# dash-robotics/perception

Measured on AMD Instinct MI355X. Metric: frames/sec (640x480 D435 cloud, plane+cluster+ICP), higher is better.
Workload: dtype f32

## Files before the change

### include/cuboid_hip.h

```cpp
#ifndef CUBOID_HIP_H
#define CUBOID_HIP_H

#include <stddef.h>
#include <stdint.h>

#ifdef __cplusplus
extern "C" {
#endif

#define CD_ABI_VERSION 4
#define CD_MAX_TEMPLATES 8
#define CD_MAX_CLUSTERS_PER_FRAME 8
#define CD_FRAME_MORE_CLUSTERS 1
#define CD_FRAME_SURFACE_GUESS 2
#define CD_FRAME_CLUSTER_GUESS 4

typedef struct cd_context cd_context;

typedef enum cd_status {
    CD_OK = 0,
    CD_ERR_INVALID_ARG = -1,
    CD_ERR_CAPACITY = -2,
    CD_ERR_DEVICE = -3,
    CD_ERR_NO_MODEL = -4,
// ... 66 lines not shown
    int32_t n_clusters;
    int32_t ransac_iterations;
    int32_t flags;
    float plane[4];
    float pad[4];
    cd_cluster_result clusters[CD_MAX_CLUSTERS_PER_FRAME];
} cd_frame_result;

void cd_default_params(cd_params* p);
int cd_abi_version(void);
int cd_struct_size(int which);

int cd_create(int device_id, int max_points, int max_frames, cd_context** out);
void cd_destroy(cd_context* ctx);
const char* cd_last_error(const cd_context* ctx);

int cd_set_template(cd_context* ctx, int slot, const void* xyz, size_t stride_bytes, int m);

int cd_template_lattice_faces(const cd_context* ctx, int slot);

int cd_template_nearest(cd_context* ctx, int slot, const void* queries, size_t stride_bytes, int n, int32_t* out_index,
                        float* out_d2);

int cd_lattice_detect(const void* xyz, size_t stride_bytes, int m, int32_t* out);

int cd_lattice_axes(const void* xyz, size_t stride_bytes, int m, int32_t* out_axis_face, float* out_axis_c);

int cd_crop_voxel(cd_context* ctx, const void* points, size_t stride_bytes, int n,
                  const cd_params* prm, float* out_xyz, uint32_t* out_rgb, int capacity,
                  int* out_n_cropped, int* out_n_voxels);

int cd_passthrough(cd_context* ctx, const void* points, size_t stride_bytes, int n, int field, double limit_min,
                   double limit_max, int negative, void* out_points, int capacity, int* out_n);

int cd_segment_plane(cd_context* ctx, const void* xyz, size_t stride_bytes, int n,
                     const cd_params* prm, float coeff[4], int32_t* inliers, int capacity,
                     int* out_n_inliers, int* out_iterations);

int cd_surface_frame(cd_context* ctx, const void* xyz, size_t stride_bytes, int n, const float table_normal[3],
                     int invert, const cd_params* prm, cd_surface_frame_result* out);

int cd_surface_batch(cd_context* ctx, const void* xyz, size_t stride_bytes, int points_per_frame, const int32_t* n_points,
                     int n_frames, const float* table_normals, int invert, const cd_params* prm, cd_surface_frame_result* out,
                     int32_t* frame_status);

int cd_surface_guess(const float Rt[16], float guess[16]);
// ... 235 lines not shown
```

### perception_amd/capi.py

```python
import ctypes as C
import os

import numpy as np

CD_ABI_VERSION = 4
CD_MAX_TEMPLATES = 8
CD_MAX_CLUSTERS_PER_FRAME = 8
CD_FRAME_MORE_CLUSTERS = 1
CD_FRAME_SURFACE_GUESS = 2
CD_FRAME_CLUSTER_GUESS = 4

CD_OK = 0
CD_ERR_INVALID_ARG = -1
CD_ERR_CAPACITY = -2
CD_ERR_DEVICE = -3
CD_ERR_NO_MODEL = -4
CD_ERR_FEW_CORRESPONDENCES = -5
CD_ERR_LEAF_TOO_SMALL = -6
CD_ERR_NO_TEMPLATE = -7

LIB_PATH = os.environ.get("CUBOID_HIP_LIB") or os.path.join(os.path.dirname(os.path.abspath(__file__)), "lib", "libcuboid_hip.so")

EXPORTED_SYMBOLS = [
    "cd_default_params", "cd_abi_version", "cd_struct_size", "cd_create", "cd_destroy", "cd_last_error",
    "cd_set_template", "cd_crop_voxel", "cd_segment_plane", "cd_extract", "cd_surface_frame", "cd_bbox_filter", "cd_cluster", "cd_icp",
    "cd_process_batch", "cd_process_frame", "cd_process_batch_device", "cd_get_cluster_results", "cd_pose_to_position_quaternion",
    "cd_bbox_corners", "cd_get_timing", "cd_get_frame_cloud", "cd_get_cluster_points", "cd_ground_plane", "cd_set_frame_guesses",
    "cd_template_lattice_faces", "cd_template_nearest", "cd_lattice_detect", "cd_lattice_axes", "cd_passthrough",
    "cd_default_depth_camera", "cd_depth_to_cloud", "cd_process_depth_batch", "cd_process_depth_batch_device",
    "cd_set_icp_max_correspondence_distance", "cd_get_icp_max_correspondence_distance", "cd_icp_correspondence_threshold",
    "cd_surface_batch", "cd_surface_guess", "cd_set_surface_distance_threshold", "cd_get_surface_distance_threshold",
    "cd_get_surface_results",
    "cd_default_color_gate_params", "cd_color_bbox_batch", "cd_color_bbox_batch_device", "cd_set_frame_bboxes", "cd_set_bbox_source",
    "cd_get_bbox_source", "cd_get_frame_bboxes",
    "cd_default_overlay_params", "cd_overlay_project", "cd_draw_boxes_batch", "cd_draw_boxes_batch_device", "cd_draw_last_results",
    "cd_draw_last_results_device",
    "cd_default_verify_params", "cd_verify_struct_size", "cd_verify_pixel", "cd_verify_box_host", "cd_verify_boxes_batch",
    "cd_verify_boxes_batch_device", "cd_verify_last_results", "cd_verify_last_results_device",
    "cd_default_color_camera", "cd_color_camera_struct_size", "cd_texture_project", "cd_depth_to_cloud_mapped",
    "cd_process_depth_batch_mapped", "cd_process_depth_batch_mapped_device",
    "cd_shape_frame_struct_size", "cd_shape_frame_host", "cd_shape_frames", "cd_template_shape_frame", "cd_shape_guess",
    "cd_get_cluster_shape_frames",
]

CD_CLOUD_VOXELS, CD_CLOUD_OBJECTS = 0, 1
CD_GUESS_NONE, CD_GUESS_PARAMS, CD_GUESS_PER_FRAME, CD_GUESS_SURFACE, CD_GUESS_CLUSTER = 0, 1, 2, 3, 4


CD_PLANE, CD_PLANE_PERPENDICULAR, CD_PLANE_PARALLEL = 0, 1, 2
CD_COLOR_NONE, CD_COLOR_RGB8 = 0, 1
CD_BBOX_PARAMS, CD_BBOX_PER_FRAME, CD_BBOX_COLOR = 0, 1, 2
CD_DRAW_ACCEPTED, CD_DRAW_ALL = 0, 1
CD_VERIFY_ACCEPTED, CD_VERIFY_ALL = 0, 1
CD_VERIFY_MISS, CD_VERIFY_AGREE, CD_VERIFY_THROUGH, CD_VERIFY_OCCLUDED, CD_VERIFY_INVALID = 0, 1, 2, 3, 4
CD_NOTEX_DROP, CD_NOTEX_KEEP = 0, 1


class CdSurfaceFrameResult(C.Structure):
    _fields_ = [("Rt", C.c_float * 16), ("coeff", (C.c_float * 4) * 3), ("midpoint", (C.c_float * 4) * 3),
                ("n_points", C.c_int32 * 3), ("iterations", C.c_int32 * 3), ("reserved", C.c_int32 * 2)]


class CdShapeFrame(C.Structure):
    _fields_ = [("n", C.c_int32), ("status", C.c_int32), ("mean", C.c_double * 3), ("axes", C.c_double * 9),
                ("var", C.c_double * 3), ("lo", C.c_double * 3), ("hi", C.c_double * 3)]
# ... 261 lines not shown
    lib.cd_icp.argtypes = [vp, C.c_int, vp, C.c_size_t, C.c_int, C.POINTER(CdParams),
                           C.POINTER(CdClusterResult), vp]
    for f in (lib.cd_process_batch, lib.cd_process_batch_device):
        f.argtypes = [vp, vp, C.c_size_t, C.c_int, C.c_int, C.POINTER(CdParams), vp, vp, vp]
    lib.cd_process_frame.argtypes = [vp, vp, C.c_size_t, C.c_int, C.POINTER(CdParams), vp, vp, vp]
    lib.cd_get_cluster_results.argtypes = [vp, C.c_int, C.c_int, C.c_int, C.POINTER(CdClusterResult), ip]
    lib.cd_pose_to_position_quaternion.argtypes = [C.POINTER(C.c_double)] * 3
    lib.cd_pose_to_position_quaternion.restype = None
    lib.cd_bbox_corners.argtypes = [C.POINTER(C.c_double), C.c_double, C.c_double, C.c_double, f32p]
    lib.cd_bbox_corners.restype = None
    lib.cd_get_timing.argtypes = [vp, C.POINTER(CdTiming)]
    lib.cd_get_frame_cloud.argtypes = [vp, C.c_int, C.c_int, vp, C.c_size_t, C.c_int, C.c_int, ip]
    lib.cd_get_cluster_points.argtypes = [vp, C.c_int, C.c_int, C.c_int, vp, C.c_size_t, C.c_int, ip]
    lib.cd_ground_plane.argtypes = [vp, vp, C.c_size_t, C.c_int, C.POINTER(CdParams), f32p, vp, C.c_int, ip, ip]
    lib.cd_set_frame_guesses.argtypes = [vp, f32p, C.c_int]
    lib.cd_surface_batch.argtypes = [vp, vp, C.c_size_t, C.c_int, i32p, C.c_int, f32p, C.c_int, C.POINTER(CdParams),
                                     C.POINTER(CdSurfaceFrameResult), i32p]
    lib.cd_surface_guess.argtypes = [f32p, f32p]
    lib.cd_set_surface_distance_threshold.argtypes = [vp, C.c_double]
    lib.cd_get_surface_distance_threshold.argtypes = [vp, C.POINTER(C.c_double)]
    lib.cd_get_surface_results.argtypes = [vp, C.c_int, C.c_int, C.POINTER(CdSurfaceFrameResult), i32p]
    lib.cd_template_lattice_faces.argtypes = [vp, C.c_int]
    lib.cd_template_nearest.argtypes = [vp, C.c_int, vp, C.c_size_t, C.c_int, vp, vp]
    lib.cd_lattice_detect.argtypes = [vp, C.c_size_t, C.c_int, vp]
    lib.cd_lattice_axes.argtypes = [vp, C.c_size_t, C.c_int, vp, vp]
    lib.cd_set_icp_max_correspondence_distance.argtypes = [vp, C.c_double]
    lib.cd_get_icp_max_correspondence_distance.argtypes = [vp, C.POINTER(C.c_double)]
    lib.cd_icp_correspondence_threshold.argtypes = [C.c_double, C.POINTER(C.c_float), ip]
    lib.cd_passthrough.argtypes = [vp, vp, C.c_size_t, C.c_int, C.c_int, C.c_double, C.c_double, C.c_int, vp, C.c_int, ip]
    lib.cd_default_depth_camera.argtypes = [C.POINTER(CdDepthCamera)]
    lib.cd_default_depth_camera.restype = None
    lib.cd_depth_to_cloud.argtypes = [vp, C.POINTER(CdDepthCamera), vp, vp, vp, C.c_size_t, C.c_int, C.c_int, ip]
    for f in (lib.cd_process_depth_batch, lib.cd_process_depth_batch_device):
        f.argtypes = [vp, C.POINTER(CdDepthCamera), vp, vp, C.c_int, C.POINTER(CdParams), vp, vp, vp]
    lib.cd_default_color_gate_params.argtypes = [C.POINTER(CdColorGateParams)]
    lib.cd_default_color_gate_params.restype = None
    for f in (lib.cd_color_bbox_batch, lib.cd_color_bbox_batch_device):
        f.argtypes = [vp, vp, C.c_int, C.c_int, C.c_int, C.POINTER(CdColorGateParams), C.POINTER(CdColorBBox)]
    lib.cd_set_frame_bboxes.argtypes = [vp, i32p, C.c_int]
    lib.cd_set_bbox_source.argtypes = [vp, C.c_int, C.POINTER(CdColorGateParams)]
    lib.cd_get_bbox_source.argtypes = [vp, ip]
    lib.cd_get_frame_bboxes.argtypes = [vp, C.c_int, C.c_int, C.POINTER(CdColorBBox)]
    dp = C.POINTER(C.c_double)
    lib.cd_default_overlay_params.argtypes = [C.POINTER(CdOverlayParams)]
    lib.cd_default_overlay_params.restype = None
    lib.cd_overlay_project.argtypes = [dp, C.POINTER(CdOverlayParams), C.POINTER(CdOverlayBox)]
# ... 467 lines not shown


def lattice_detect(xyz):
    lib = load_library()
    a, stride, m = _points(xyz)
    out = np.zeros((8, 5), np.int32)
    nf = lib.cd_lattice_detect(_ptr(a), stride, m, _ptr(out))
    if nf < 0:
        raise CuboidError(nf, "cd_lattice_detect")
    return [tuple(int(v) for v in out[f]) for f in range(nf)]


def lattice_axes(xyz):
    lib = load_library()
    a, stride, m = _points(xyz)
    face = np.zeros(3, np.int32)
    c = np.zeros(3, np.float32)
    r = lib.cd_lattice_axes(_ptr(a), stride, m, _ptr(face), _ptr(c))
    if r < 0:
        raise CuboidError(r, "cd_lattice_axes")
    return int(r), [int(v) for v in face], c


def icp_correspondence_threshold(d):
    lib = load_library()
    f, b = C.c_float(), C.c_int()
    st = lib.cd_icp_correspondence_threshold(float("inf") if d is None else float(d), C.byref(f), C.byref(b))
    if st != CD_OK:
        raise CuboidError(st, "cd_icp_correspondence_threshold")
    return f.value, int(b.value)


def surface_guess(Rt):
    lib = load_library()
    a = np.ascontiguousarray(Rt, np.float32).reshape(16)
    g = np.zeros(16, np.float32)
    f32 = C.POINTER(C.c_float)
    st = lib.cd_surface_guess(a.ctypes.data_as(f32), g.ctypes.data_as(f32))
    if st != CD_OK:
        raise CuboidError(st, "cd_surface_guess: non-finite input")
    return g.reshape(4, 4)


def shape_frame_host(xyz):
    lib = load_library()
    a = np.asarray(xyz, np.float32)
# ... 82 lines not shown
```

### perception_amd/csrc/entries.hip

```cpp
#include "context.hpp"
#include "host_math.hpp"

namespace {
int cd_crop_voxel_impl(cd_context* c, const void* points, size_t stride, int n, const cd_params* p, float* out_xyz,
                  uint32_t* out_rgb, int capacity, int* out_n_cropped, int* out_n_voxels) {
    invalidate_last(c);
    int st = check_params(c, p);
    if (st) return st;
    if (!points || !out_xyz || n < 0 || stride < 12 || (stride & 3)) return fail(c, CD_ERR_INVALID_ARG, "bad arguments");
    if (n > c->N) return fail(c, CD_ERR_CAPACITY, "more points than the context capacity");
    if (out_n_cropped) *out_n_cropped = 0;
    if (out_n_voxels) *out_n_voxels = 0;
    if (n == 0) return CD_OK;
    st = ensure_input(c, (size_t)n * stride);
    if (st) return st;
    HIPCHK(c, hipMemcpyAsync(c->d_in, points, (size_t)n * stride, hipMemcpyHostToDevice, c->stream));
    st = stage_crop_voxel(c, c->d_in, stride, n, 1, p, nullptr);
    if (st) return st;
    st = sync_fs(c, 1);
    if (st) return st;
    const FrameState& s = c->h_fs[0];
    if (out_n_cropped) *out_n_cropped = s.n_cropped;
    if (s.status != CD_OK) return fail(c, s.status, "voxel grid: leaf size too small for the input extent");
    if (s.n_v > capacity) return fail(c, CD_ERR_CAPACITY, "output capacity too small");
// ... 411 lines not shown
}
int cd_bbox_filter(cd_context* c, const void* xyz, size_t stride, int n, const double P[12], const int32_t rect[4], int32_t* out_indices, int capacity, int* out_n) {
    return with_scan_retry(c, [&] { return cd_bbox_filter_impl(c, xyz, stride, n, P, rect, out_indices, capacity, out_n); });
}
int cd_extract(cd_context* c, const void* points, size_t stride, int n, const int32_t* indices, int n_indices, int negative, void* out_points, int capacity, int* out_n) {
    return with_scan_retry(c, [&] { return cd_extract_impl(c, points, stride, n, indices, n_indices, negative, out_points, capacity, out_n); });
}
int cd_passthrough(cd_context* c, const void* points, size_t stride, int n, int field, double limit_min, double limit_max, int negative, void* out_points, int capacity, int* out_n) {
    return with_scan_retry(c, [&] { return cd_passthrough_impl(c, points, stride, n, field, limit_min, limit_max, negative, out_points, capacity, out_n); });
}
int cd_cluster(cd_context* c, const void* xyz, size_t stride, int n, const cd_params* p, int32_t* labels, int32_t* sizes, int sizes_capacity, int* out_k) {
    return with_scan_retry(c, [&] { return cd_cluster_impl(c, xyz, stride, n, p, labels, sizes, sizes_capacity, out_k); });
}
int cd_icp(cd_context* c, int slot, const void* src_xyz, size_t stride, int n, const cd_params* p, cd_cluster_result* out, float* aligned) {
    return with_scan_retry(c, [&] { return cd_icp_impl(c, slot, src_xyz, stride, n, p, out, aligned); });
}
int cd_shape_frames(cd_context* c, const void* xyz, size_t stride, const int32_t* offsets, int n_sets, cd_shape_frame* out) {
    return with_scan_retry(c, [&] { return cd_shape_frames_impl(c, xyz, stride, offsets, n_sets, out); });
}
int cd_ground_plane(cd_context* c, const void* points, size_t stride, int n, const cd_params* p, float coeff[4], void* out_records, int capacity, int* out_n, int* out_n_inliers) {
    return with_scan_retry(c, [&] { return cd_ground_plane_impl(c, points, stride, n, p, coeff, out_records, capacity, out_n, out_n_inliers); });
}
}
```

### perception_amd/csrc/k_icp_lat.hip

```cpp
#include "kernels.hpp"
#include "icp_solve.hpp"

namespace cd {

struct LatFaces {
    int nface;
    unsigned m0[LAT_MAX_FACES], m1[LAT_MAX_FACES], m2[LAT_MAX_FACES];
    float c[LAT_MAX_FACES];
    int nx, ny, nz, tox, toy, toz;
    float ox, oy, oz, ivx, ivy, ivz;
    int axes;
    int afx, afy, afz;
    float cax, cay, caz;
};

__device__ __forceinline__ void lat_faces_load(const IcpLattice* __restrict__ L, LatFaces& F) {
    F.nface = L->nface;
#pragma unroll
    for (int f = 0; f < LAT_MAX_FACES; ++f) { F.m0[f] = L->m0[f]; F.m1[f] = L->m1[f]; F.m2[f] = L->m2[f]; F.c[f] = L->c[f]; }
    F.nx = L->n[0]; F.ny = L->n[1]; F.nz = L->n[2]; F.tox = L->toff[0]; F.toy = L->toff[1]; F.toz = L->toff[2];
    F.ox = L->noi[0]; F.oy = L->noi[1]; F.oz = L->noi[2]; F.ivx = L->inv[0]; F.ivy = L->inv[1]; F.ivz = L->inv[2];
    F.axes = L->axes_distinct;
    F.afx = L->axis_face[0]; F.afy = L->axis_face[1]; F.afz = L->axis_face[2];
    asm("v_mov_b32 %0, %1" : "=v"(F.cax) : "s"(L->axis_c[0]));
// ... 201 lines not shown
#else
#define LAT_T(k)
#endif

template <int SHIFT>
struct LatFix {
    static constexpr unsigned long long C = ((unsigned long long)(1023 + 52 - SHIFT) << 52) | (1ull << 51);
    static __device__ __forceinline__ unsigned long long bits(float v) {
        return (unsigned long long)__double_as_longlong(__dadd_rn((double)v, __longlong_as_double((long long)C)));
    }
};
static_assert(LatFix<32>::C == 0x4138000000000000ull && LatFix<36>::C == 0x40f8000000000000ull, "constants of lat_fix");
static_assert(FIX_SHIFT == 32 && FIX_SHIFT_D2 == 36, "k_icp_lat's moment sums are written for these scales");

struct LatSlot {
    int k, src_off, n, tslot;
    int phase;
    int gen;
    int ready;
    int pad;
};
enum { LAT_ITER = 0, LAT_FIT = 1, LAT_EMPTY = 2 };

#ifndef CD_LAT_WAVES_PER_EU
#define CD_LAT_WAVES_PER_EU 4
#endif
template <int CPW, int WPC, bool BOUNDED>
__global__ void __launch_bounds__(CPW * WPC * WAVE, CD_LAT_WAVES_PER_EU)
k_icp_lat(int nitems, const int* __restrict__ order, const IcpCluster* __restrict__ cl, IcpState* __restrict__ st,
          unsigned long long* __restrict__ accf, const IcpLattice* __restrict__ lats, float4* __restrict__ src,
          const float4* __restrict__ src0, int* __restrict__ queue, unsigned long long* __restrict__ busy,
          unsigned long long* __restrict__ busy_out, IcpParams prm, IcpBound bnd) {
    __shared__ float4 s_tab[CPW][LAT_MAX_TAB];
    __shared__ int4 s_face[CPW][2 * LAT_MAX_FACES];
    __shared__ unsigned long long s_acc[CPW][16];
    __shared__ IcpState s_so[CPW];
    __shared__ LatSlot s_slot[CPW];
    __shared__ int s_flags[2];
    __shared__ unsigned s_nv[BOUNDED ? CPW : 1];
    const int lane = threadIdx.x & 63, wave = threadIdx.x >> 6;
    const int slot = wave / WPC, sub = wave % WPC;
    const long long wg_t0 = wall_clock64();
    auto refill = [&](int s) {
        LatSlot& sl = s_slot[s];
        for (int i = 0; i < 16; ++i) s_acc[s][i] = 0ull;
        if constexpr (BOUNDED) s_nv[s] = 0u;
// ... 110 lines not shown
                unsigned long long S[16];
#pragma unroll
                for (int i = 0; i < 16; ++i) S[i] = 0ull;
                float4 pnext = pts[min((sub << 6) + lane, n - 1)], p0next = pts0[min((sub << 6) + lane, n - 1)];
                for (int pss = sub; pss < npass; pss += WPC) {
                    const int myq = (pss << 6) + lane;
                    const bool act = myq < n;
                    const float4 p = pnext, p0 = p0next;
                    pnext = pts[min(((pss + WPC) << 6) + lane, n - 1)];
                    p0next = pts0[min(((pss + WPC) << 6) + lane, n - 1)];
                    float ox, oy, oz;
                    xform(T, p.x, p.y, p.z, ox, oy, oz);
                    if (act) pts[myq] = make_float4(ox, oy, oz, p.w);
                    float qx, qy, qz;
                    xform(Tf, p0.x, p0.y, p0.z, qx, qy, qz);
                    const LatHit h = F.axes ? lat_nearest_axes<false>(tab, face, F, qx, qy, qz)
                                            : (nf3 ? lat_nearest<false, 3>(tab, face, F, qx, qy, qz) : lat_nearest<false, LAT_MAX_FACES>(tab, face, F, qx, qy, qz));
                    if (act) S[0] += h.d < 16384.f ? LatFix<FIX_SHIFT_D2>::bits(h.d) : (unsigned long long)fixq(h.d, FIX_SHIFT_D2) + LatFix<FIX_SHIFT_D2>::C;
                }
                if (sub < npass) wave_fold_to_lds(S, 1, s_acc[slot]);
            }
        }
        LAT_T(0)
        __syncthreads();
        LAT_T(1)
        if (threadIdx.x == 0) s_flags[1] = 0;
        if (threadIdx.x < CPW) {
            const int s = threadIdx.x;
            LatSlot& sl = s_slot[s];
            const int nv = BOUNDED && sl.phase == LAT_ITER ? (int)s_nv[s] : sl.n;
            const unsigned long long off = (unsigned long long)nv * LatFix<FIX_SHIFT>::C, off_d = (unsigned long long)nv * LatFix<FIX_SHIFT_D2>::C;
            if (sl.phase == LAT_ITER && sl.ready) {
                for (int i = 0; i < 15; ++i) s_acc[s][i] -= off;
                s_acc[s][15] -= off_d;
                if (icp_step<BOUNDED>(s_so[s], s_acc[s], nv, prm)) sl.phase = LAT_FIT;
                for (int i = 0; i < 16; ++i) s_acc[s][i] = 0ull;
                if constexpr (BOUNDED) s_nv[s] = 0u;
                sl.ready = 0;
            } else if (sl.phase == LAT_FIT) {
                s_so[s].done = 1;
                st[2 * (size_t)sl.k] = s_so[s];
                st[2 * (size_t)sl.k + 1] = s_so[s];
                accf[sl.k] = s_acc[s][0] - off_d;
                refill(s);
                if (sl.phase != LAT_EMPTY) s_flags[1] = 1;
            }
        }
        if (threadIdx.x == 0) {
            int all_empty = 1;
            for (int s = 0; s < CPW; ++s) all_empty &= s_slot[s].phase == LAT_EMPTY ? 1 : 0;
            s_flags[0] = all_empty;
        }
        LAT_T(2)
        __syncthreads();
        LAT_T(3)
#ifdef CD_LAT_TIMERS
        tph[4] += 1;
#endif
        if (s_flags[0]) break;
    }
#ifdef CD_LAT_TIMERS
    if (threadIdx.x == 0) for (int i = 0; i < 6; ++i) atomicAdd(&g_lat_stats[i], (unsigned long long)tph[i]);
#endif
    if (threadIdx.x == 0 && busy) {
        atomicAdd(busy, (unsigned long long)(wall_clock64() - wg_t0) * (unsigned long long)(CPW * WPC));
        if (busy_out) {
            __threadfence();
            if (atomicAdd(queue + 1, 1) == (int)gridDim.x - 1) {
                __threadfence();
                *busy_out = atomicAdd(busy, 0ull);
            }
        }
    }
}

__device__ __forceinline__ bool lat_same_bits(float a, float b) { return __float_as_uint(a) == __float_as_uint(b); }

__global__ void __launch_bounds__(BLOCK) k_lat_nn(const IcpLattice* __restrict__ L, const float4* __restrict__ q, int n, int* __restrict__ out_idx,
                                                  float* __restrict__ out_d2) {
    __shared__ float4 s_tab[LAT_MAX_TAB];
    __shared__ int4 s_face[2 * LAT_MAX_FACES];
    LatFaces F;
// ... 47 lines not shown
```

Baseline: 199,700.

## Parallelize ICP 3x3 SVD step across 16 lanes per slot in lattice kernel

Replaces the single-thread-per-slot ICP update (SVD of the 3x3 cross-covariance plus convergence test) with a row-parallel version where 16 lanes per slot each own one accumulator entry and cooperate via cross-lane reads. It also adds fast sqrt/rcp paths with exact rounding fixups for arguments of at least one, and moves the all-empty check out of a serialized thread-0 loop so every thread evaluates it after the barrier. The aim is to shorten the serial tail between the two barriers in each ICP iteration. The cost is extra code complexity and a bit-exactness burden, covered by a new batch-solve entry point and an exhaustive test harness.

```diff
diff --git a/include/cuboid_hip.h b/include/cuboid_hip.h
--- a/include/cuboid_hip.h
+++ b/include/cuboid_hip.h
@@ -112,6 +112,10 @@
 int cd_template_nearest(cd_context* ctx, int slot, const void* queries, size_t stride_bytes, int n, int32_t* out_index,
                         float* out_d2);
 
+int cd_icp_solve_batch(int k, const uint64_t* sums, const int32_t* n, const void* states_in, int max_iter, double trans_eps,
+                       double rel_mse, double rot_thr, double abs_mse, int bounded, void* states_row, void* states_lane,
+                       int32_t* done, uint64_t* unary);
+
 int cd_lattice_detect(const void* xyz, size_t stride_bytes, int m, int32_t* out);
 
 int cd_lattice_axes(const void* xyz, size_t stride_bytes, int m, int32_t* out_axis_face, float* out_axis_c);
diff --git a/perception_amd/capi.py b/perception_amd/capi.py
--- a/perception_amd/capi.py
+++ b/perception_amd/capi.py
@@ -41,6 +41,7 @@
     "cd_process_depth_batch_mapped", "cd_process_depth_batch_mapped_device",
     "cd_shape_frame_struct_size", "cd_shape_frame_host", "cd_shape_frames", "cd_template_shape_frame", "cd_shape_guess",
     "cd_get_cluster_shape_frames",
+    "cd_icp_solve_batch",
 ]
 
 CD_CLOUD_VOXELS, CD_CLOUD_OBJECTS = 0, 1
@@ -348,6 +349,7 @@
     lib.cd_get_surface_results.argtypes = [vp, C.c_int, C.c_int, C.POINTER(CdSurfaceFrameResult), i32p]
     lib.cd_template_lattice_faces.argtypes = [vp, C.c_int]
     lib.cd_template_nearest.argtypes = [vp, C.c_int, vp, C.c_size_t, C.c_int, vp, vp]
+    lib.cd_icp_solve_batch.argtypes = [C.c_int, vp, vp, vp, C.c_int, C.c_double, C.c_double, C.c_double, C.c_double, C.c_int, vp, vp, vp, vp]
     lib.cd_lattice_detect.argtypes = [vp, C.c_size_t, C.c_int, vp]
     lib.cd_lattice_axes.argtypes = [vp, C.c_size_t, C.c_int, vp, vp]
     lib.cd_set_icp_max_correspondence_distance.argtypes = [vp, C.c_double]
@@ -861,6 +863,27 @@
     return int(r), [int(v) for v in face], c
 
 
+ICP_STATE = np.dtype([("Tfinal", np.float32, 16), ("T", np.float32, 16), ("prev_mse", np.float64), ("iters", np.int32),
+                      ("done", np.int32), ("converged", np.int32), ("status", np.int32)])
+
+
+def icp_solve_batch(sums, n, states, max_iter=50, trans_eps=1e-8, rel_mse=1e-6, rot_thr=None, abs_mse=1e-12, bounded=False, unary=False):
+    lib = load_library()
+    sums = np.ascontiguousarray(sums, np.uint64).reshape(-1, 16)
+    k = sums.shape[0]
+    n = np.ascontiguousarray(n, np.int32).reshape(k)
+    states = np.ascontiguousarray(states, ICP_STATE).reshape(k)
+    out_row, out_lane = np.zeros(k, ICP_STATE), np.zeros(k, ICP_STATE)
+    done = np.zeros((k, 2), np.int32)
+    un = np.zeros(6, np.uint64) if unary else None
+    st = lib.cd_icp_solve_batch(k, _ptr(sums), _ptr(n), _ptr(states), int(max_iter), float(trans_eps), float(rel_mse),
+                                float(1.0 - trans_eps if rot_thr is None else rot_thr), float(abs_mse), int(bool(bounded)),
+                                _ptr(out_row), _ptr(out_lane), _ptr(done), None if un is None else _ptr(un))
+    if st != CD_OK:
+        raise CuboidError(st, "cd_icp_solve_batch")
+    return out_row, out_lane, done, un
+
+
 def icp_correspondence_threshold(d):
     lib = load_library()
     f, b = C.c_float(), C.c_int()
diff --git a/perception_amd/csrc/entries.hip b/perception_amd/csrc/entries.hip
--- a/perception_amd/csrc/entries.hip
+++ b/perception_amd/csrc/entries.hip
@@ -1,5 +1,6 @@
 #include "context.hpp"
 #include "host_math.hpp"
+#include "icp_solve_row.hpp"
 
 namespace {
 int cd_crop_voxel_impl(cd_context* c, const void* points, size_t stride, int n, const cd_params* p, float* out_xyz,
@@ -457,3 +458,89 @@
     return with_scan_retry(c, [&] { return cd_ground_plane_impl(c, points, stride, n, p, coeff, out_records, capacity, out_n, out_n_inliers); });
 }
 }
+
+template <bool BOUNDED>
+__global__ void __launch_bounds__(WAVE) k_icp_solve_batch(int k, const unsigned long long* __restrict__ sums, const int* __restrict__ n,
+                                                           const IcpState* __restrict__ in, IcpParams prm, IcpState* __restrict__ out_row,
+                                                           IcpState* __restrict__ out_lane, int* __restrict__ done) {
+    __shared__ IcpState s_row[4], s_one[4];
+    __shared__ unsigned long long s_sums[4][16];
+    const int tid = (int)threadIdx.x, r = tid >> 4, l = tid & 15;
+    const int rec = (int)blockIdx.x * 4 + r;
+    if (rec >= k) return;
+    if (l == 0) { s_row[r] = in[rec]; s_one[r] = in[rec]; }
+    s_sums[r][l] = sums[(size_t)rec * 16 + l];
+    const int nn = n[rec];
+    RowLanes row(tid);
+    RowLanes::V<unsigned long long> a;
+    a.v = s_sums[r][l];
+    const int d_row = icp_step_row<BOUNDED>(row, s_row[r], a, nn, prm);
+    if (l == 0) {
+        const int d_one = icp_step<BOUNDED>(s_one[r], s_sums[r], nn, prm);
+        out_row[rec] = s_row[r];
+        out_lane[rec] = s_one[r];
+        done[2 * rec] = d_row;
+        done[2 * rec + 1] = d_one;
+    }
+}
+__global__ void __launch_bounds__(BLOCK) k_unary_exhaustive(unsigned long long* __restrict__ res) {
+    unsigned long long bad_s = 0, bad_r = 0, first_s = ~0ull, first_r = ~0ull;
+    const unsigned lo = 0x3f800000u, hi = 0x7f800000u, rcp_end = 0x7e800000u;
+    for (unsigned long long b = lo + (unsigned long long)blockIdx.x * BLOCK + threadIdx.x; b <= hi; b += (unsigned long long)gridDim.x * BLOCK) {
+        const float x = __uint_as_float((unsigned)b);
+        if (__float_as_uint(sqrt_ge1(x)) != __float_as_uint(sqrtf(x))) { bad_s += 1; first_s = first_s < b ? first_s : b; }
+        if (b < rcp_end) {
+            if (__float_as_uint(rcp_ge1(x)) != __float_as_uint(1.0f / x)) { bad_r += 1; first_r = first_r < b ? first_r : b; }
+            const unsigned long long bn = b | 0x80000000ull;
+            if (__float_as_uint(rcp_ge1(-x)) != __float_as_uint(1.0f / -x)) { bad_r += 1; first_r = first_r < bn ? first_r : bn; }
+        }
+    }
+    if (bad_s) { atomicAdd(&res[0], bad_s); atomicMin(&res[1], first_s); }
+    if (bad_r) { atomicAdd(&res[2], bad_r); atomicMin(&res[3], first_r); }
+}
+
+extern "C" int cd_icp_solve_batch(int k, const uint64_t* sums, const int32_t* n, const void* states_in, int max_iter, double trans_eps,
+                                  double rel_mse, double rot_thr, double abs_mse, int bounded, void* states_row, void* states_lane,
+                                  int32_t* done, uint64_t* unary) {
+    static_assert(sizeof(IcpState) == 152, "the record layout cuboid_hip.h documents");
+    if (k < 0 || (k > 0 && (!sums || !n || !states_in || !states_row || !states_lane || !done))) return CD_ERR_INVALID_ARG;
+    unsigned long long *d_sums = nullptr, *d_res = nullptr;
+    int *d_n = nullptr, *d_done = nullptr;
+    IcpState *d_in = nullptr, *d_row = nullptr, *d_lane = nullptr;
+    bool ok = true;
+    auto chk = [&](hipError_t e) { ok = ok && e == hipSuccess; return ok; };
+    if (k > 0) {
+        const size_t kk = (size_t)k;
+        if (chk(hipMalloc(&d_sums, kk * 128)) && chk(hipMalloc(&d_n, kk * 4)) && chk(hipMalloc(&d_done, kk * 8)) && chk(hipMalloc(&d_in, kk * sizeof(IcpState))) &&
+            chk(hipMalloc(&d_row, kk * sizeof(IcpState))) && chk(hipMalloc(&d_lane, kk * sizeof(IcpState))) &&
+            chk(hipMemcpy(d_sums, sums, kk * 128, hipMemcpyHostToDevice)) && chk(hipMemcpy(d_n, n, kk * 4, hipMemcpyHostToDevice)) &&
+            chk(hipMemcpy(d_in, states_in, kk * sizeof(IcpState), hipMemcpyHostToDevice))) {
+            IcpParams prm;
+            std::memset(&prm, 0, sizeof(prm));
+            prm.max_iter = max_iter; prm.trans_eps = trans_eps; prm.rel_mse = rel_mse; prm.rot_thr = rot_thr; prm.abs_mse = abs_mse;
+            const int grid = (k + 3) / 4;
+            if (bounded) hipLaunchKernelGGL(k_icp_solve_batch<true>, dim3(grid), dim3(WAVE), 0, 0, k, d_sums, d_n, d_in, prm, d_row, d_lane, d_done);
+            else hipLaunchKernelGGL(k_icp_solve_batch<false>, dim3(grid), dim3(WAVE), 0, 0, k, d_sums, d_n, d_in, prm, d_row, d_lane, d_done);
+            chk(hipGetLastError());
+            chk(hipDeviceSynchronize());
+            chk(hipMemcpy(states_row, d_row, kk * sizeof(IcpState), hipMemcpyDeviceToHost));
+            chk(hipMemcpy(states_lane, d_lane, kk * sizeof(IcpState), hipMemcpyDeviceToHost));
+            chk(hipMemcpy(done, d_done, kk * 8, hipMemcpyDeviceToHost));
+        }
+    }
+    if (ok && unary) {
+        const unsigned long long init[4] = {0ull, ~0ull, 0ull, ~0ull};
+        if (chk(hipMalloc(&d_res, sizeof(init))) && chk(hipMemcpy(d_res, init, sizeof(init), hipMemcpyHostToDevice))) {
+            hipLaunchKernelGGL(k_unary_exhaustive, dim3(4096), dim3(BLOCK), 0, 0, d_res);
+            chk(hipGetLastError());
+            chk(hipDeviceSynchronize());
+            chk(hipMemcpy(unary, d_res, sizeof(init), hipMemcpyDeviceToHost));
+        }
+        if (ok) {
+            unary[4] = CD_ROW_SQRT_GE1;
+            unary[5] = CD_ROW_RCP_GE1;
+        }
+    }
+    (void)hipFree(d_sums); (void)hipFree(d_n); (void)hipFree(d_done); (void)hipFree(d_in); (void)hipFree(d_row); (void)hipFree(d_lane); (void)hipFree(d_res);
+    return ok ? CD_OK : CD_ERR_DEVICE;
+}
diff --git a/perception_amd/csrc/icp_solve_row.hpp b/perception_amd/csrc/icp_solve_row.hpp
--- /dev/null
+++ b/perception_amd/csrc/icp_solve_row.hpp
@@ -0,0 +1,294 @@
+#pragma once
+#include "icp_solve.hpp"
+
+namespace cd {
+
+#ifndef CD_ROW_SQRT_GE1
+#define CD_ROW_SQRT_GE1 1
+#endif
+#ifndef CD_ROW_RCP_GE1
+#define CD_ROW_RCP_GE1 1
+#endif
+
+constexpr float RCP_GE1_END = 0x1p126f;
+__device__ __forceinline__ float sqrt_ge1(float x) {
+#if defined(__HIP_DEVICE_COMPILE__) && CD_ROW_SQRT_GE1
+    float s = __builtin_amdgcn_sqrtf(x);
+    const float sd = __uint_as_float(__float_as_uint(s) - 1u), su = __uint_as_float(__float_as_uint(s) + 1u);
+    const float ed = __builtin_fmaf(-sd, s, x), eu = __builtin_fmaf(-su, s, x);
+    s = ed <= 0.f ? sd : s;
+    s = eu > 0.f ? su : s;
+    return s;
+#else
+#ifdef CD_ROW_POISON
+    if (x < 1.0f) return 12345.f;
+#endif
+    return sqrtf(x);
+#endif
+}
+__device__ __forceinline__ float rcp_ge1(float x) {
+#if defined(__HIP_DEVICE_COMPILE__) && CD_ROW_RCP_GE1
+    float r = __builtin_amdgcn_rcpf(x);
+    r = __builtin_fmaf(__builtin_fmaf(-x, r, 1.0f), r, r);
+    r = __builtin_fmaf(__builtin_fmaf(-x, r, 1.0f), r, r);
+    return r;
+#else
+#ifdef CD_ROW_POISON
+    if (fabsf(x) < 1.0f || fabsf(x) >= RCP_GE1_END) return 12345.f;
+#endif
+    return 1.0f / x;
+#endif
+}
+__device__ __forceinline__ void row_rotation(float m00, float m01, float m10, float m11, Rot& rot1, Rot& j_right) {
+    const float t = m00 + m11, d = m10 - m01;
+    float s1 = 1.0f, x3 = 1.0f, y = 1.0f;
+    if (t == 0.f) {
+        rot1.c = 0.f;
+        rot1.s = d > 0.f ? 1.f : -1.f;
+    } else {
+        const float u = d / t;
+        s1 = sqrt_ge1(1.0f + u * u);
+        rot1.c = rcp_ge1(s1);
+        rot1.s = rot1.c * u;
+    }
+    {
+        const float n00 = rot1.c * m00 + rot1.s * m10, n01 = rot1.c * m01 + rot1.s * m11;
+        const float n11 = -rot1.s * m01 + rot1.c * m11;
+        if (n01 == 0.f) {
+            j_right = {1.f, 0.f};
+        } else {
+            y = n01;
+            const float tau = (n00 - n11) / (2.0f * fabsf(y));
+            const float w = sqrt_ge1(tau * tau + 1.0f);
+            x3 = tau > 0.f ? tau + w : tau - w;
+            const float tt = rcp_ge1(x3);
+            const float n = rcp_ge1(sqrt_ge1(tt * tt + 1.0f));
+            const float at = fabsf(tt);
+            j_right.s = ((tt > 0.f) != (y < 0.f) ? -at : at) * n;
+            j_right.c = n;
+        }
+    }
+    if (!(s1 < RCP_GE1_END && fabsf(x3) < RCP_GE1_END && fabsf(y) < __builtin_inff())) {
+        if (t == 0.f) {
+            rot1.c = 0.f;
+            rot1.s = d > 0.f ? 1.f : -1.f;
+        } else {
+            const float u = d / t;
+            rot1.c = 1.0f / sqrtf(1.0f + u * u);
+            rot1.s = rot1.c * u;
+        }
+        const float n00 = rot1.c * m00 + rot1.s * m10, n01 = rot1.c * m01 + rot1.s * m11;
+        const float n11 = -rot1.s * m01 + rot1.c * m11;
+        j_right = make_jacobi(n00, n01, n11);
+    }
+}
+
+template <int N> struct RowIdx { static constexpr int value = N; };
+
+template <bool BOUNDED, class R>
+__device__ __forceinline__ int icp_step_row(R& row, IcpState& so, const typename R::template V<unsigned long long>& a, int n, const IcpParams& prm) {
+    using VF = typename R::template V<float>;
+    using VD = typename R::template V<double>;
+    if (BOUNDED && n < ICP_MIN_CORR) {
+        row.each([&](int l) {
+            so.T[l] = (l % 5 == 0) ? 1.f : 0.f;
+            if (l == 0) so.converged = 0;
+        });
+        return 1;
+    }
+    VD m;
+    VF mf;
+    row.each([&](int l) {
+        m(l) = unfix(a(l), l == 15 ? FIX_SHIFT_D2 : FIX_SHIFT) / (double)n;
+        mf(l) = (float)m(l);
+    });
+    VF sg;
+    row.each([&](int l) {
+        const int k = (l >= 6 && l < 15) ? l - 6 : 0, ia = k / 3, ib = k - 3 * ia;
+        const double mqa = row.read(m, 3 + ia), mpb = row.read(m, ib);
+        sg(l) = (float)(m(l) - mqa * mpb);
+    });
+    float sigma[3][3];
+#pragma unroll
+    for (int i = 0; i < 3; ++i)
+#pragma unroll
+        for (int j = 0; j < 3; ++j) sigma[i][j] = row.read(sg, 6 + 3 * i + j);
+    const float precision = 2.0f * 1.1920928955078125e-07f;
+    const float consider_zero = 2.0f * 1.401298464324817e-45f;
+    float scale = 0.f;
+#pragma unroll
+    for (int i = 0; i < 3; ++i)
+#pragma unroll
+        for (int j = 0; j < 3; ++j) scale = fmaxf(scale, fabsf(sigma[i][j]));
+    if (scale == 0.f) scale = 1.f;
+    VF wl;
+    row.each([&](int l) { wl(l) = sg(l) / scale; });
+    float W[3][3];
+#pragma unroll
+    for (int i = 0; i < 3; ++i)
+#pragma unroll
+        for (int j = 0; j < 3; ++j) W[i][j] = row.read(wl, 6 + 3 * i + j);
+    VF X[3];
+    row.each([&](int l) {
+        X[0](l) = (l & 3) == 0 ? 1.f : 0.f;
+        X[1](l) = (l & 3) == 1 ? 1.f : 0.f;
+        X[2](l) = (l & 3) == 2 ? 1.f : 0.f;
+    });
+    bool finished = false;
+    auto pair = [&](auto P, auto Q) {
+        constexpr int p = decltype(P)::value, q = decltype(Q)::value;
+        const float thr = fmaxf(consider_zero, precision * fmaxf(fabsf(W[p][p]), fabsf(W[q][q])));
+        if (fabsf(W[p][q]) > thr || fabsf(W[q][p]) > thr) {
+            finished = false;
+            Rot rot1, j_right;
+            row_rotation(W[p][p], W[p][q], W[q][p], W[q][q], rot1, j_right);
+            const Rot j_left = rot_mul(rot1, rot_T(j_right));
+            apply_left(W, p, q, j_left);
+            apply_right(W, p, q, j_right);
+            const Rot j_u = rot_T(j_left);
+            row.each([&](int l) {
+                const float c = l < 4 ? j_u.c : j_right.c, s = l < 4 ? j_u.s : j_right.s;
+                const float x = X[p](l), y = X[q](l);
+                X[p](l) = c * x - s * y;
+                X[q](l) = s * x + c * y;
+            });
+        }
+    };
+    for (int sweep = 0; sweep < 64 && !finished; ++sweep) {
+        finished = true;
+        pair(RowIdx<1>(), RowIdx<0>());
+        pair(RowIdx<2>(), RowIdx<0>());
+        pair(RowIdx<2>(), RowIdx<1>());
+    }
+    float S[3];
+#pragma unroll
+    for (int i = 0; i < 3; ++i) {
+        const float av = fabsf(W[i][i]);
+        S[i] = av;
+        if (av != 0.f) {
+            const float f = W[i][i] / av;
+            row.each([&](int l) { if (l < 4) X[i](l) *= f; });
+        }
+    }
+#define CD_ROW_SWAP_COLS(ca, cb)                                                                   \
+    {                                                                                              \
+        const float t_ = S[ca]; S[ca] = S[cb]; S[cb] = t_;                                         \
+        row.each([&](int l) { const float u_ = X[ca](l); X[ca](l) = X[cb](l); X[cb](l) = u_; });   \
+    }
+    {
+        int pos = 0;
+        float mxv = S[0];
+        if (S[1] > mxv) { mxv = S[1]; pos = 1; }
+        if (S[2] > mxv) { mxv = S[2]; pos = 2; }
+        if (mxv != 0.f) {
+            if (pos == 1) CD_ROW_SWAP_COLS(0, 1)
+            else if (pos == 2) CD_ROW_SWAP_COLS(0, 2)
+            if (S[2] > S[1]) CD_ROW_SWAP_COLS(1, 2)
+        }
+    }
+#undef CD_ROW_SWAP_COLS
+#pragma unroll
+    for (int i = 0; i < 3; ++i) S[i] *= scale;
+    float sd[3] = {1.f, 1.f, 1.f};
+    if (det3(sigma) < 0.f) sd[2] = -1.f;
+    int rank = 0;
+#pragma unroll
+    for (int i = 0; i < 3; ++i)
+        if (!(fabsf(S[i]) <= fabsf(S[0]) * 1e-5f)) ++rank;
+    if (rank == 2) {
+        float Uf[3][3], Vf[3][3];
+#pragma unroll
+        for (int r = 0; r < 3; ++r)
+#pragma unroll
+            for (int c = 0; c < 3; ++c) {
+                Uf[r][c] = row.read(X[c], r);
+                Vf[r][c] = row.read(X[c], 4 + r);
+            }
+        sd[0] = 1.f; sd[1] = 1.f;
+        sd[2] = (det3(Uf) * det3(Vf) > 0.f) ? 1.f : -1.f;
+    }
+    VF rr;
+    row.each([&](int l) {
+        const int i = l >> 2, j = l & 3;
+        const float u0 = row.read(X[0], i), u1 = row.read(X[1], i), u2 = row.read(X[2], i);
+        const float v0 = row.read(X[0], 4 + j), v1 = row.read(X[1], 4 + j), v2 = row.read(X[2], 4 + j);
+        rr(l) = ((u0 * sd[0]) * v0 + (u1 * sd[1]) * v1) + (u2 * sd[2]) * v2;
+    });
+    VF t;
+    row.each([&](int l) {
+        const int i = l >> 2, j = l & 3, b = l & 12;
+        const float r0 = row.read(rr, b), r1 = row.read(rr, b + 1), r2 = row.read(rr, b + 2);
+        const float p0 = row.read(mf, 0), p1 = row.read(mf, 1), p2 = row.read(mf, 2), qi = row.read(mf, 3 + (i < 3 ? i : 0));
+        const float tr = qi - ((r0 * p0 + r1 * p1) + r2 * p2);
+        t(l) = i == 3 ? (j == 3 ? 1.f : 0.f) : (j == 3 ? tr : rr(l));
+    });
+    VF c;
+    row.each([&](int l) {
+        const int j = l & 3, b = l & 12;
+        const float t0 = row.read(t, b), t1 = row.read(t, b + 1), t2 = row.read(t, b + 2), t3 = row.read(t, b + 3);
+        c(l) = ((t0 * so.Tfinal[j] + t1 * so.Tfinal[4 + j]) + t2 * so.Tfinal[8 + j]) + t3 * so.Tfinal[12 + j];
+    });
+    const int iters = so.iters + 1;
+    int done = 0;
+    bool mse_seen = false;
+    double mse = 0.0;
+    if (iters >= prm.max_iter) {
+        done = 1;
+    } else {
+        const float T0 = row.read(t, 0), T5 = row.read(t, 5), T10 = row.read(t, 10), T3 = row.read(t, 3), T7 = row.read(t, 7), T11 = row.read(t, 11);
+        const double cos_angle = 0.5 * (double)(((T0 + T5) + T10) - 1.0f);
+        const double translation_sqr = (double)((T3 * T3 + T7 * T7) + T11 * T11);
+        if (cos_angle >= prm.rot_thr && translation_sqr <= prm.trans_eps) {
+            done = 1;
+        } else {
+            mse = row.read(m, 15);
+            const double prev = so.prev_mse;
+            if (fabs(mse - prev) < prm.abs_mse) done = 1;
+            else if (fabs(mse - prev) / prev < prm.rel_mse) done = 1;
+            mse_seen = true;
+        }
+    }
+    row.each([&](int l) {
+        so.Tfinal[l] = c(l);
+        so.T[l] = t(l);
+        if (l == 0) {
+            so.iters = iters;
+            if (mse_seen) so.prev_mse = mse;
+            so.converged = done;
+        }
+    });
+    return done;
+}
+
+#ifdef __HIPCC__
+struct RowLanes {
+    template <class T>
+    struct V {
+        T v;
+        __device__ __forceinline__ T& operator()(int) { return v; }
+        __device__ __forceinline__ const T& operator()(int) const { return v; }
+    };
+    int l, base;
+    __device__ __forceinline__ explicit RowLanes(int thread) {
+        const int lane = thread & 63;
+        l = lane & 15;
+        base = (lane & 48) << 2;
+    }
+    template <class F> __device__ __forceinline__ void each(F&& f) { f(l); }
+    __device__ __forceinline__ int read_word(int w, int src) const {
+#ifdef __HIP_DEVICE_COMPILE__
+        return __builtin_amdgcn_ds_bpermute(base + (src << 2), w);
+#else
+        return w;
+#endif
+    }
+    __device__ __forceinline__ float read(const V<float>& x, int src) const { return __int_as_float(read_word(__float_as_int(x.v), src)); }
+    __device__ __forceinline__ double read(const V<double>& x, int src) const {
+        const long long b = __double_as_longlong(x.v);
+        const unsigned lo = (unsigned)read_word((int)(unsigned)b, src), hi = (unsigned)read_word((int)(unsigned)((unsigned long long)b >> 32), src);
+        return __longlong_as_double((long long)(((unsigned long long)hi << 32) | lo));
+    }
+};
+#endif
+
+}
diff --git a/perception_amd/csrc/icp_solve_row_check.cpp b/perception_amd/csrc/icp_solve_row_check.cpp
--- /dev/null
+++ b/perception_amd/csrc/icp_solve_row_check.cpp
@@ -0,0 +1,256 @@
+#include <cmath>
+#include <cstdio>
+#include <cstdlib>
+#include <cstring>
+#include <thread>
+#include <vector>
+
+#include "common.hpp"
+namespace cd {
+long long fixq(float v, int shift);
+unsigned long long fixq_fast(float v, int shift);
+}
+float __fmul_rn(float a, float b);
+#define CD_ROW_POISON 1
+#include "icp_solve_row.hpp"
+
+using namespace cd;
+
+struct RowHost {
+    template <class T>
+    struct V {
+        T v[16];
+        T& operator()(int l) { return v[l]; }
+        const T& operator()(int l) const { return v[l]; }
+    };
+    template <class F> void each(F&& f) { for (int l = 0; l < 16; ++l) f(l); }
+    template <class T> T read(const V<T>& x, int src) const { return x.v[src]; }
+};
+
+struct Rng {
+    uint64_t s;
+    uint64_t next() {
+        uint64_t z = (s += 0x9E3779B97F4A7C15ull);
+        z = (z ^ (z >> 30)) * 0xBF58476D1CE4E5B9ull;
+        z = (z ^ (z >> 27)) * 0x94D049BB133111EBull;
+        return z ^ (z >> 31);
+    }
+    double uni(double lo, double hi) { return lo + (hi - lo) * ((double)(next() >> 11) * (1.0 / 9007199254740992.0)); }
+    int below(int n) { return (int)(next() % (uint64_t)n); }
+};
+
+struct Counts { long long sets = 0, stop = 0, limit = 0, eps = 0, abs_ = 0, rel = 0, open = 0, rank2 = 0, bad = 0; };
+
+static unsigned long long fix(double v, int shift) { return (unsigned long long)std::llrint(std::ldexp(v, shift)); }
+static void sums_from(int n, const double mp[3], const double mq[3], const double sg[9], double mse, unsigned long long A[16]) {
+    const double k = n > 0 ? n : 1;
+    for (int a = 0; a < 3; ++a) { A[a] = fix(k * mp[a], FIX_SHIFT); A[3 + a] = fix(k * mq[a], FIX_SHIFT); }
+    for (int a = 0; a < 3; ++a)
+        for (int b = 0; b < 3; ++b) A[6 + 3 * a + b] = fix(k * (sg[3 * a + b] + mq[a] * mp[b]), FIX_SHIFT);
+    A[15] = fix(k * mse, FIX_SHIFT_D2);
+}
+static void rotation(Rng& g, double R[9]) {
+    const double rx = g.uni(-3.2, 3.2), ry = g.uni(-3.2, 3.2), rz = g.uni(-3.2, 3.2);
+    const double cx = cos(rx), sx = sin(rx), cy = cos(ry), sy = sin(ry), cz = cos(rz), sz = sin(rz);
+    const double M[9] = {cz * cy, cz * sy * sx - sz * cx, cz * sy * cx + sz * sx, sz * cy, sz * sy * sx + cz * cx, sz * sy * cx - cz * sx, -sy, cy * sx, cy * cx};
+    std::memcpy(R, M, sizeof(M));
+}
+static void mul3(const double A[9], const double B[9], double C[9]) {
+    for (int i = 0; i < 3; ++i)
+        for (int j = 0; j < 3; ++j) C[3 * i + j] = A[3 * i] * B[j] + A[3 * i + 1] * B[3 + j] + A[3 * i + 2] * B[6 + j];
+}
+static IcpState state_in(Rng& g, int iters) {
+    IcpState s;
+    std::memset(&s, 0, sizeof(s));
+    double R[9];
+    rotation(g, R);
+    for (int i = 0; i < 3; ++i) {
+        for (int j = 0; j < 3; ++j) s.Tfinal[4 * i + j] = (float)R[3 * i + j];
+        s.Tfinal[4 * i + 3] = (float)g.uni(-1.0, 1.0);
+    }
+    s.Tfinal[15] = 1.f;
+    for (int i = 0; i < 16; ++i) s.T[i] = (float)g.uni(-1.0, 1.0);
+    s.prev_mse = g.below(8) == 0 ? 1.7976931348623157e308 : g.uni(0.0, 1e-3);
+    s.iters = iters;
+    s.status = 7;
+    return s;
+}
+
+template <bool BOUNDED>
+static bool one(const unsigned long long A[16], int n, const IcpState& in, const IcpParams& prm, Counts& c, const char* what) {
+    IcpState ref = in, got = in;
+    const int dref = icp_step<BOUNDED>(ref, A, n, prm);
+    RowHost row;
+    RowHost::V<unsigned long long> a;
+    for (int l = 0; l < 16; ++l) a(l) = A[l];
+    const int dgot = icp_step_row<BOUNDED>(row, got, a, n, prm);
+    c.sets += 1;
+    if (BOUNDED && n < ICP_MIN_CORR) c.stop += 1;
+    else if (ref.iters >= prm.max_iter) c.limit += 1;
+    else if (dref && std::memcmp(&ref.prev_mse, &in.prev_mse, 8) == 0) c.eps += 1;
+    else if (dref && std::fabs(ref.prev_mse - in.prev_mse) < prm.abs_mse) c.abs_ += 1;
+    else if (dref) c.rel += 1;
+    else c.open += 1;
+    if (dref == dgot && std::memcmp(&ref, &got, sizeof(IcpState)) == 0) return true;
+    if (c.bad++ == 0) {
+        std::fprintf(stderr, "DIFFERENT (%s, bounded %d, n %d): done %d / %d\n", what, (int)BOUNDED, n, dref, dgot);
+        for (int i = 0; i < 16; ++i) std::fprintf(stderr, "  A[%2d] %016llx  T %a / %a  Tfinal %a / %a\n", i, A[i], ref.T[i], got.T[i], ref.Tfinal[i], got.Tfinal[i]);
+        std::fprintf(stderr, "  prev_mse %a / %a iters %d / %d converged %d / %d\n", ref.prev_mse, got.prev_mse, ref.iters, got.iters, ref.converged, got.converged);
+    }
+    return false;
+}
+static bool both(const unsigned long long A[16], int n, const IcpState& in, const IcpParams& prm, Counts& c, const char* what) {
+    const bool x = one<false>(A, n, in, prm, c, what), y = one<true>(A, n, in, prm, c, what);
+    return x && y;
+}
+
+static IcpParams params(int kind) {
+    IcpParams p;
+    std::memset(&p, 0, sizeof(p));
+    p.max_iter = 50;
+    p.trans_eps = 1e-8; p.rot_thr = 1.0 - 1e-8; p.rel_mse = 1e-6; p.abs_mse = 1e-12;
+    if (kind == 1) { p.trans_eps = 1e-3; p.rot_thr = 1.0 - 1e-3; }
+    if (kind == 2) { p.abs_mse = 1e-5; }
+    if (kind == 3) { p.rel_mse = 0.5; }
+    if (kind == 4) { p.max_iter = 3; }
+    return p;
+}
+
+static void random_sets(uint64_t seed, long long count, Counts& c) {
+    Rng g{seed};
+    for (long long it = 0; it < count; ++it) {
+        const int kind = g.below(10);
+        int n = 3 + g.below(2000);
+        double mp[3], mq[3], sg[9];
+        for (int a = 0; a < 3; ++a) { mp[a] = g.uni(-1.0, 1.0); mq[a] = g.uni(-1.0, 1.0); }
+        for (double& v : sg) v = g.uni(-1.0, 1.0);
+        double mse = g.uni(0.0, 1e-3);
+        unsigned long long A[16];
+        if (kind == 1) { const double s = std::pow(10.0, g.uni(-9.0, 3.0)); for (double& v : sg) v *= s; }
+        if (kind == 2) { sg[3] = sg[1]; sg[6] = sg[2]; sg[7] = sg[5]; }
+        if (kind == 3) for (double& v : sg) if (g.below(2)) v = 0.0;
+        if (kind == 4 || kind == 5 || kind == 6) {
+            double U[9], V[9], D[9] = {0}, UD[9];
+            rotation(g, U); rotation(g, V);
+            if (kind == 4) D[0] = D[4] = D[8] = g.uni(0.01, 1.0);
+            if (kind == 5) { D[0] = g.uni(0.1, 1.0); D[4] = g.uni(0.01, 0.1) * (g.below(2) ? 1.0 : -1.0); D[8] = 0.0; for (int a = 0; a < 3; ++a) mp[a] = mq[a] = 0.0; n = 1; }
+            if (kind == 6) { D[0] = g.uni(0.01, 1.0); D[4] = g.uni(0.01, 1.0); D[8] = g.uni(-1.0, 1.0); std::memcpy(V, U, sizeof(U)); for (int a = 0; a < 3; ++a) mq[a] = mp[a] + g.uni(-1e-5, 1e-5); }
+            mul3(U, D, UD);
+            double Vt[9];
+            for (int i = 0; i < 3; ++i) for (int j = 0; j < 3; ++j) Vt[3 * i + j] = V[3 * j + i];
+            mul3(UD, Vt, sg);
+        }
+        if (kind == 7) {
+            n = 3 + g.below(40);
+            double R[9], tr[3] = {g.uni(-0.05, 0.05), g.uni(-0.05, 0.05), g.uni(-0.05, 0.05)};
+            rotation(g, R);
+            if (g.below(2)) { const double I[9] = {1, 0, 0, 0, 1, 0, 0, 0, 1}; std::memcpy(R, I, sizeof(I)); }
+            for (auto& v : A) v = 0ull;
+            for (int i = 0; i < n; ++i) {
+                const float p[3] = {(float)g.uni(-0.2, 0.2), (float)g.uni(-0.1, 0.1), (float)g.uni(0.3, 0.9)};
+                float q[3];
+                for (int a = 0; a < 3; ++a) q[a] = (float)(R[3 * a] * p[0] + R[3 * a + 1] * p[1] + R[3 * a + 2] * p[2] + tr[a] + g.uni(-1e-4, 1e-4));
+                const float d2 = ((q[0] - p[0]) * (q[0] - p[0]) + (q[1] - p[1]) * (q[1] - p[1])) + (q[2] - p[2]) * (q[2] - p[2]);
+                for (int a = 0; a < 3; ++a) {
+                    A[a] += fix(p[a], FIX_SHIFT); A[3 + a] += fix(q[a], FIX_SHIFT);
+                    for (int b = 0; b < 3; ++b) A[6 + 3 * a + b] += fix(q[a] * p[b], FIX_SHIFT);
+                }
+                A[15] += fix(d2, FIX_SHIFT_D2);
+            }
+        } else {
+            sums_from(n, mp, mq, sg, mse, A);
+        }
+        const IcpParams prm = params(g.below(5));
+        IcpState in = state_in(g, g.below(6));
+        if (g.below(4) == 0) in.prev_mse = mse * (1.0 + g.uni(-1e-6, 1e-6));
+        const int nb = g.below(50) == 0 ? g.below(4) : n;
+        if (nb != n && kind != 7) sums_from(nb, mp, mq, sg, mse, A);
+        if (kind == 7 && nb != n) continue;
+        if (kind == 5) c.rank2 += 1;
+        both(A, nb, in, prm, c, "random");
+    }
+}
+
+static void structured(Counts& c) {
+    Rng g{77};
+    const double Z[3] = {0, 0, 0};
+    const double mats[][9] = {
+        {0, 0, 0, 0, 0, 0, 0, 0, 0},
+        {0.5, 0, 0, 0, 0, 0, 0, 0, 0},
+        {0, 0, 0.25, 0, 0, 0, 0, 0, 0},
+        {0.5, 0, 0, 0, 0.25, 0, 0, 0, 0},
+        {0.5, 0, 0, 0, -0.25, 0, 0, 0, 0},
+        {0, 0.5, 0, 0.25, 0, 0, 0, 0, 0},
+        {0.5, 0, 0, 0, 0.25, 0, 0, 0, -0.125},
+        {-0.5, 0, 0, 0, -0.25, 0, 0, 0, -0.125},
+        {0.5, 0.25, 0, 0.125, -0.5, 0, 0, 0, 0.25},
+        {0.5, 0.25, 0, -0.25, -0.5, 0, 0, 0, 0.25},
+        {0.5, 0.25, 0, 0.25, -0.5, 0, 0, 0, 0.25},
+        {0, 0.125, 0, 0, 0.5, 0, 0, 0, 0.25},
+        {0.25, 0, 0, 0.125, 0, 0, 0, 0, 0.5},
+        {0.5, 0, 0, 0, 0.5, 0, 0, 0, 0.5},
+        {0.125, 0, 0, 0, 0.25, 0, 0, 0, 0.5},
+        {0.25, 0, 0, 0, 0.5, 0, 0, 0, 0.125},
+        {1, 1, 1, 1, 1, 1, 1, 1, 1},
+        {1, 2, 3, 4, 5, 6, 7, 8, 9},
+        {2147483647.0, 0, 0, 0, 1.0 / 4294967296.0, 0, 0, 0, 1},
+        {1.0 / 4294967296.0, 1.0 / 4294967296.0, 0, 0, 1.0 / 4294967296.0, 0, 0, 0, 0},
+    };
+    for (const auto& sg : mats)
+        for (int kind = 0; kind < 5; ++kind)
+            for (int n : {1, 2, 3, 4, 1000}) {
+                unsigned long long A[16];
+                sums_from(n, Z, Z, sg, 1e-4, A);
+                for (int iters : {0, 2, 49}) both(A, n, state_in(g, iters), params(kind), c, "structured");
+            }
+    const unsigned long long ends[] = {0ull, 1ull, ~0ull, 1ull << 62, (unsigned long long)(-(1ll << 62)), 0x7fffffffffffffffull, 0x8000000000000000ull};
+    for (int rep = 0; rep < 4000; ++rep) {
+        unsigned long long A[16];
+        for (auto& v : A) v = rep < 200 ? ends[g.below(7)] : (g.below(3) ? g.next() : ends[g.below(7)]);
+        const int ns[] = {0, 1, 2, 3, 7, 2147483647, -1};
+        both(A, ns[g.below(7)], state_in(g, g.below(4)), params(g.below(5)), c, "extreme");
+    }
+    for (int rep = 0; rep < 200; ++rep) {
+        double U[9], D[9] = {0}, UD[9], Ut[9], sg[9], mp[3] = {g.uni(-1, 1), g.uni(-1, 1), g.uni(-1, 1)};
+        rotation(g, U);
+        D[0] = g.uni(0.1, 1.0); D[4] = g.uni(0.1, 1.0); D[8] = g.uni(0.1, 1.0);
+        mul3(U, D, UD);
+        for (int i = 0; i < 3; ++i) for (int j = 0; j < 3; ++j) Ut[3 * i + j] = U[3 * j + i];
+        mul3(UD, Ut, sg);
+        unsigned long long A[16];
+        sums_from(500, mp, mp, sg, 1e-4, A);
+        for (int kind = 0; kind < 5; ++kind) {
+            IcpState in = state_in(g, 1);
+            both(A, 500, in, params(kind), c, "identity");
+            in.prev_mse = unfix(A[15], FIX_SHIFT_D2) / 500.0;
+            both(A, 500, in, params(kind), c, "same mse");
+            in.prev_mse *= 1.0 + 1e-9;
+            both(A, 500, in, params(kind), c, "close mse");
+        }
+        double mq[3] = {mp[0] + 0.01, mp[1], mp[2]};
+        sums_from(500, mp, mq, sg, 1e-4, A);
+        IcpState in = state_in(g, 1);
+        in.prev_mse = unfix(A[15], FIX_SHIFT_D2) / 500.0;
+        both(A, 500, in, params(0), c, "same mse, moving");
+        in.prev_mse *= 1.0 + 1e-9;
+        both(A, 500, in, params(0), c, "close mse, moving");
+    }
+}
+
+int main(int argc, char** argv) {
+    const long long total = argc > 1 ? std::atoll(argv[1]) : 10000000ll;
+    const int nthreads = 8;
+    std::vector<Counts> cs(nthreads + 1);
+    structured(cs[nthreads]);
+    std::vector<std::thread> th;
+    for (int i = 0; i < nthreads; ++i)
+        th.emplace_back([&, i] { random_sets(20190409ull + 1000003ull * (uint64_t)i, total / nthreads + (i < total % nthreads ? 1 : 0), cs[i]); });
+    for (auto& t : th) t.join();
+    Counts c;
+    for (const Counts& x : cs) {
+        c.sets += x.sets; c.stop += x.stop; c.limit += x.limit; c.eps += x.eps; c.abs_ += x.abs_; c.rel += x.rel; c.open += x.open; c.rank2 += x.rank2; c.bad += x.bad;
+    }
+    if (c.bad) { std::printf("FAILED %lld of %lld\n", c.bad, c.sets); return 1; }
+    std::printf("ok %lld %lld %lld %lld %lld %lld %lld %lld\n", c.sets, c.stop, c.limit, c.eps, c.abs_, c.rel, c.open, c.rank2);
+    return 0;
+}
diff --git a/perception_amd/csrc/k_icp_lat.hip b/perception_amd/csrc/k_icp_lat.hip
--- a/perception_amd/csrc/k_icp_lat.hip
+++ b/perception_amd/csrc/k_icp_lat.hip
@@ -1,5 +1,5 @@
 #include "kernels.hpp"
-#include "icp_solve.hpp"
+#include "icp_solve_row.hpp"
 
 namespace cd {
 
@@ -247,6 +247,9 @@
 };
 enum { LAT_ITER = 0, LAT_FIT = 1, LAT_EMPTY = 2 };
 
+#ifndef CD_LAT_SOLVE_ROW
+#define CD_LAT_SOLVE_ROW 1
+#endif
 #ifndef CD_LAT_WAVES_PER_EU
 #define CD_LAT_WAVES_PER_EU 4
 #endif
@@ -403,9 +406,38 @@
             }
         }
         LAT_T(0)
+        if (threadIdx.x == 0) s_flags[1] = 0;
         __syncthreads();
         LAT_T(1)
-        if (threadIdx.x == 0) s_flags[1] = 0;
+#if CD_LAT_SOLVE_ROW
+        const int tid = (int)threadIdx.x | s_flags[0];
+        if (tid < CPW * 16) {
+            const int s = tid >> 4, l = tid & 15;
+            LatSlot& sl = s_slot[s];
+            const int phase = sl.phase, ready = sl.ready;
+            const int nv = BOUNDED && phase == LAT_ITER ? (int)s_nv[s] : sl.n;
+            const unsigned long long off = (unsigned long long)nv * LatFix<FIX_SHIFT>::C, off_d = (unsigned long long)nv * LatFix<FIX_SHIFT_D2>::C;
+            if (phase == LAT_ITER && ready) {
+                RowLanes row(tid);
+                RowLanes::V<unsigned long long> a;
+                a.v = s_acc[s][l] - (l == 15 ? off_d : off);
+                const int done = icp_step_row<BOUNDED>(row, s_so[s], a, nv, prm);
+                s_acc[s][l] = 0ull;
+                if (l == 0) {
+                    if (done) sl.phase = LAT_FIT;
+                    if constexpr (BOUNDED) s_nv[s] = 0u;
+                    sl.ready = 0;
+                }
+            } else if (phase == LAT_FIT && l == 0) {
+                s_so[s].done = 1;
+                st[2 * (size_t)sl.k] = s_so[s];
+                st[2 * (size_t)sl.k + 1] = s_so[s];
+                accf[sl.k] = s_acc[s][0] - off_d;
+                refill(s);
+                if (sl.phase != LAT_EMPTY) s_flags[1] = 1;
+            }
+        }
+#else
         if (threadIdx.x < CPW) {
             const int s = threadIdx.x;
             LatSlot& sl = s_slot[s];
@@ -427,18 +459,17 @@
                 if (sl.phase != LAT_EMPTY) s_flags[1] = 1;
             }
         }
-        if (threadIdx.x == 0) {
-            int all_empty = 1;
-            for (int s = 0; s < CPW; ++s) all_empty &= s_slot[s].phase == LAT_EMPTY ? 1 : 0;
-            s_flags[0] = all_empty;
-        }
+#endif
         LAT_T(2)
         __syncthreads();
         LAT_T(3)
 #ifdef CD_LAT_TIMERS
         tph[4] += 1;
 #endif
-        if (s_flags[0]) break;
+        int all_empty = 1;
+#pragma unroll
+        for (int s = 0; s < CPW; ++s) all_empty &= s_slot[s].phase == LAT_EMPTY ? 1 : 0;
+        if (all_empty) break;
     }
 #ifdef CD_LAT_TIMERS
     if (threadIdx.x == 0) for (int i = 0; i < 6; ++i) atomicAdd(&g_lat_stats[i], (unsigned long long)tph[i]);
```

Result: faster. 207,300, median of 6 (+3.8%).
